# thunlp/OpenMatch

Hardware: NVIDIA H100
Metric: queries/sec top-1000 over 8.8M x 768 corpus (higher is better)
Workload: dtype f16

## Files before the change

openmatch_b200/csrc/encoder.cu:

```cuda
#include <math.h>
#include <stdlib.h>
#include <string.h>

#include <algorithm>
#include <new>
#include <set>
#include <string>
#include <vector>

#include "common.h"
#include "gemm.cuh"

namespace om {

constexpr int kAttnCols = 64;
constexpr int kMaxL = 128;
constexpr int kMaxLongL = 512;
constexpr float kLog2e = 1.4426950408889634f;

__device__ __forceinline__ float rcp_approx(float x) {
  float y;
  asm("rcp.approx.ftz.f32 %0, %1;" : "=f"(y) : "f"(x));
  return y;
}
// ... 94 lines not shown
      store_direct(held, out, ldo, row, held_col, M);
      have = 0;
    }
  }
  __device__ __forceinline__ void finish() {
    if (in_flight && (threadIdx.x & 31) == 0) bulk_wait_group0();
  }
};

template <int ACT>
struct EpiBiasActBf16 {
  CUtensorMap tm_out;
  __nv_bfloat16* out;
  int64_t ldo;
  const float* bias;
  int M, N;
  RowNorm norm;
  static constexpr int kPasses = 1;
  static constexpr bool kPrefetch = false;
  __host__ __device__ static constexpr int smem_bytes(int epi_warps) { return epi_warps * StagedBf16::kBytesPerWarp; }
  struct State {
    StagedBf16 stage;
    float rstd, rm;
  };
  __device__ __forceinline__ void bind(State& s, uint8_t* smem, int epi_tid) const { s.stage.bind(smem, epi_tid); }
  __device__ __forceinline__ void finish(State& s) const { s.stage.finish(); }
  __device__ __forceinline__ void begin(State& s, int row, int, int) const {
    s.stage.have = 0;
    norm.get(row, M, s.rstd, s.rm);
  }
  __device__ __forceinline__ void end(State& s, int row) const { s.stage.flush_tail(out, ldo, row, M); }
  __device__ __forceinline__ void chunk(State& s, int row, int col0, const float (&v)[32]) const {
    if (col0 >= N) return;
    uint32_t packed[16];
    float bv[32];
#pragma unroll
    for (int j = 0; j < 8; ++j) {
      const float4 t = bias ? __ldg(reinterpret_cast<const float4*>(bias + col0) + j) : make_float4(0.f, 0.f, 0.f, 0.f);
      bv[4 * j] = t.x, bv[4 * j + 1] = t.y, bv[4 * j + 2] = t.z, bv[4 * j + 3] = t.w;
    }
    const float2 rs = splat2(s.rstd);
#pragma unroll
    for (int i = 0; i < 32; i += 2) {
      float2 ab = fma2(rs, make_float2(v[i], v[i + 1]), make_float2(bv[i], bv[i + 1]));
      if (ACT == ACT_GELU) {
        ab = gelu_erf2(ab);
      } else if (ACT == ACT_RELU) {
        ab.x = fmaxf(ab.x, 0.f);
        ab.y = fmaxf(ab.y, 0.f);
      }
      packed[i >> 1] = pack_bf16x2(ab.x, ab.y);
    }
    s.stage.push(packed, &tm_out, row, col0);
  }
};

struct EpiQKV {
  CUtensorMap tm_qk;
  __nv_bfloat16* qk;
  __nv_bfloat16* vt;
  int64_t ldv;
  const float* bias;
  int M, I2;
  int valid_rows;
  RowNorm norm;
  static constexpr int kPasses = 1;
  static constexpr bool kPrefetch = false;
  __host__ __device__ static constexpr int smem_bytes(int epi_warps) { return epi_warps * StagedBf16::kBytesPerWarp; }
  struct State {
    int vcol;
    StagedBf16 stage;
    float rstd, rm;
  };
  __device__ __forceinline__ void bind(State& s, uint8_t* smem, int epi_tid) const { s.stage.bind(smem, epi_tid); }
  __device__ __forceinline__ void finish(State& s) const { s.stage.finish(); }
  __device__ __forceinline__ void begin(State& s, int row, int, int) const {
    s.vcol = (row / valid_rows) * 128 + row % valid_rows;
    s.stage.have = 0;
    norm.get(row, M, s.rstd, s.rm);
  }
  __device__ __forceinline__ void end(State& s, int row) const { s.stage.flush_tail(qk, I2, row, M); }
  __device__ __forceinline__ void chunk(State& s, int row, int col0, const float (&v)[32]) const {
    if (col0 >= I2 + (I2 >> 1)) return;
    float bv[32];
#pragma unroll
    for (int j = 0; j < 8; ++j) {
      const float4 t = bias ? __ldg(reinterpret_cast<const float4*>(bias + col0) + j) : make_float4(0.f, 0.f, 0.f, 0.f);
      bv[4 * j] = t.x, bv[4 * j + 1] = t.y, bv[4 * j + 2] = t.z, bv[4 * j + 3] = t.w;
    }
    const float rstd = s.rstd;
    if (col0 < I2) {
      uint32_t packed[16];
#pragma unroll
      for (int i = 0; i < 32; i += 2)
        packed[i >> 1] = pack_bf16x2(fmaf(rstd, v[i], bv[i]), fmaf(rstd, v[i + 1], bv[i + 1]));
      s.stage.push(packed, &tm_qk, row, col0);
    } else if (row < M) {
      __nv_bfloat16* dst = vt + static_cast<int64_t>(col0 - I2) * ldv + s.vcol;
#pragma unroll
      for (int i = 0; i < 32; ++i)
        dst[static_cast<int64_t>(i) * ldv] = __float2bfloat16(fmaf(rstd, v[i], bv[i]));
    }
  }
};

struct EpiResidNorm {
  CUtensorMap tm_s;
  CUtensorMap tm_xb;
  const float* bias;
  RowNorm norm;
  const float* gamma;
  const float* beta;
  float* stats_out;
  int parts;
  int M, N;
  int bn;
  static constexpr int kPasses = 1;
  static constexpr bool kPrefetch = true;
  static constexpr int kF32Tile = 4096, kBf16Tile = 2048, kPerWarp = kF32Tile + kBf16Tile;
  static constexpr int kMaxN = 1024;
  __host__ __device__ static constexpr int smem_bytes(int epi_warps) { return epi_warps * kPerWarp + 1024 + 2 * kMaxN * 4; }
  struct State {
    uint8_t* f32tile;
    uint8_t* bf16tile;
    uint64_t* bars;
    const float* gsm;
    const float* bsm;
    uint32_t parity;
    int slot;
    int group;
    float rstd, rm, rsum, rsq;
  };
  __device__ __forceinline__ void bind(State& s, uint8_t* smem, int epi_tid) const {
    const int w = epi_tid >> 5, nw = blockDim.x / 32 - kGemmProducerThreads / 32;
    s.f32tile = smem + w * kF32Tile;
    s.bf16tile = smem + nw * kF32Tile + w * kBf16Tile;
    s.bars = reinterpret_cast<uint64_t*>(smem + nw * kPerWarp) + w;
    s.parity = 0;
    s.group = w >> 2;
    if ((epi_tid & 31) == 0) {
      mbar_init(&s.bars[0], 1);
      fence_barrier_init();
    }
    float* gs = reinterpret_cast<float*>(smem + nw * kPerWarp + 1024);
    float* bs = gs + kMaxN;
    const bool ln = norm.stats != nullptr;
    for (int c = epi_tid; c < N; c += nw * 32) {
      gs[c] = ln ? gamma[c] : 1.f;
      bs[c] = (bias ? bias[c] : 0.f) + (ln ? beta[c] : 0.f);
    }
    s.gsm = gs;
    s.bsm = bs;
    named_bar_sync(1, nw * 32);
  }
  __device__ __forceinline__ void finish(State&) const {
    if ((threadIdx.x & 31) == 0) bulk_wait_group0();
  }
  __device__ __forceinline__ void begin(State& s, int row, int m_blk, int n_blk) const {
    norm.get(row, M, s.rstd, s.rm);
    s.rsum = 0.f;
    s.rsq = 0.f;
    s.slot = n_blk * parts + s.group;
    if (bn > 0 && (threadIdx.x & 31) == 0) {
      const int num_n = (N + bn - 1) / bn, num_m = (M + kBlockM - 1) / kBlockM;
      const int next = m_blk * num_n + n_blk + static_cast<int>(gridDim.x);
      if (next < num_m * num_n) {
        const int nm = next / num_n, nn = next - nm * num_n;
        const int row0 = row + (nm - m_blk) * kBlockM;
        const int cols = bn / parts;
#pragma unroll 1
        for (int c = 0; c < cols; c += 32) tma_prefetch_l2_2d(&tm_s, nn * bn + s.group * cols + c, row0);
      }
    }
  }
  __device__ __forceinline__ void request(State& s, int row0, int col0) const {
    bulk_wait_group_read0();
    mbar_arrive_expect_tx(&s.bars[0], kF32Tile);
    tma_load_2d(s.f32tile, &tm_s, &s.bars[0], col0, row0);
  }
  __device__ __forceinline__ void prefetch(State& s, int row, int col0) const {
    if (col0 >= N) return;
    if ((threadIdx.x & 31) == 0) request(s, row, col0);
  }
  __device__ __forceinline__ void end(State& s, int row) const {
    if (row < M)
      *reinterpret_cast<float2*>(stats_out + (static_cast<int64_t>(row) * kStatParts + s.slot) * 2) = make_float2(s.rsum, s.rsq);
  }
  __device__ __forceinline__ void chunk(State& s, int row, int col0, const float (&v)[32], int next_col0) const {
    if (col0 >= N) return;
    const int lane = threadIdx.x & 31;
    mbar_wait_warp(&s.bars[0], s.parity, 20);
    s.parity ^= 1u;
    uint8_t* mine = s.f32tile + lane * 128;
    uint8_t* mineb = s.bf16tile + lane * 64;
    const float rstd = s.rstd, nrm = -s.rm;
    const float4* gp = reinterpret_cast<const float4*>(s.gsm + col0);
    const float4* bp = reinterpret_cast<const float4*>(s.bsm + col0);
    float rsum = 0.f, rsq = 0.f;
#pragma unroll
    for (int p = 0; p < 8; ++p) {
      float4* slot = reinterpret_cast<float4*>(mine + ((p ^ (lane & 7)) << 4));
      const float4 r = *slot;
      const float4 g = gp[p], bb = bp[p];
      float4 o;
      o.x = fmaf(r.x, rstd * g.x, fmaf(nrm, g.x, bb.x)) + v[4 * p];
      o.y = fmaf(r.y, rstd * g.y, fmaf(nrm, g.y, bb.y)) + v[4 * p + 1];
      o.z = fmaf(r.z, rstd * g.z, fmaf(nrm, g.z, bb.z)) + v[4 * p + 2];
      o.w = fmaf(r.w, rstd * g.w, fmaf(nrm, g.w, bb.w)) + v[4 * p + 3];
      *slot = o;
      rsum += (o.x + o.y) + (o.z + o.w);
      rsq = fmaf(o.x, o.x, fmaf(o.y, o.y, fmaf(o.z, o.z, fmaf(o.w, o.w, rsq))));
      uint2* hb = reinterpret_cast<uint2*>(mineb + ((((p >> 1) ^ ((lane >> 1) & 3)) << 4) | ((p & 1) << 3)));
      *hb = make_uint2(pack_bf16x2(o.x, o.y), pack_bf16x2(o.z, o.w));
    }
    if (row < M) {
      s.rsum += rsum;
      s.rsq += rsq;
    }
    fence_proxy_async_smem();
    __syncwarp();
    if (lane == 0) {
      tma_store_2d(&tm_s, s.f32tile, col0, row);
      tma_store_2d(&tm_xb, s.bf16tile, col0, row);
      bulk_commit_group();
      if (next_col0 >= 0 && next_col0 < N) request(s, row, next_col0);
    }
  }
};

constexpr int kMaxVec = 8;

template <bool RMS>
__device__ __forceinline__ void norm_row(float4 (&v)[kMaxVec], int nvec, int H, float eps) {
  float s = 0.f;
  if (!RMS) {
#pragma unroll
    for (int j = 0; j < kMaxVec; ++j)
      if (j < nvec) s += (v[j].x + v[j].y) + (v[j].z + v[j].w);
#pragma unroll
    for (int o = 16; o > 0; o >>= 1) s += __shfl_xor_sync(0xffffffffu, s, o);
  }
  const float mean = RMS ? 0.f : s / H;
  float q = 0.f;
#pragma unroll
  for (int j = 0; j < kMaxVec; ++j)
    if (j < nvec) {
      const float a = v[j].x - mean, b = v[j].y - mean, c = v[j].z - mean, d = v[j].w - mean;
      q += (a * a + b * b) + (c * c + d * d);
    }
#pragma unroll
  for (int o = 16; o > 0; o >>= 1) q += __shfl_xor_sync(0xffffffffu, q, o);
  const float rstd = rsqrtf(q / H + eps);
#pragma unroll
  for (int j = 0; j < kMaxVec; ++j)
// ... 917 lines not shown
  if (kind == OM_DEVICE) OM_CUDA(cudaDeviceSynchronize());
  float* staged = dst_f32;
  float* tmp = nullptr;
  if (!staged) {
    OM_CUDA(cudaMalloc(&tmp, count * sizeof(float)));
    staged = tmp;
  }
  cudaError_t err =
      cudaMemcpy(staged, data, count * sizeof(float), kind == OM_HOST ? cudaMemcpyHostToDevice : cudaMemcpyDeviceToDevice);
  if (err == cudaSuccess && dst_bf16) {
    f32_to_bf16_kernel<<<static_cast<int>(std::min<size_t>((count + 255) / 256, 4096)), 256>>>(staged, dst_bf16,
                                                                                              (int64_t)count);
    err = cudaGetLastError();
  }
  if (err == cudaSuccess) err = cudaDeviceSynchronize();
  if (tmp) cudaFree(tmp);
  if (err != cudaSuccess) return fail(OM_ECUDA, "weight upload failed: %s", cudaGetErrorString(err));
  return 0;
}

template <int DH>
cudaError_t attn_opt_in() {
  const auto smem = cudaFuncAttributeMaxDynamicSharedMemorySize;
  cudaError_t err = cudaFuncSetAttribute(attn_stream_kernel<DH>, smem, kAttnStreamSmemBytes);
  if (err == cudaSuccess) err = cudaFuncSetAttribute(attn_long_kernel<DH>, smem, kAttnLongSmemBytes);
  if (err == cudaSuccess) err = cudaFuncSetAttribute(attn_kernel<DH>, smem, kAttnSmemBytes);
  return err;
}

template <int DH>
void attn_launch(const CUtensorMap& tmQK, const CUtensorMap& tmVt, const AttnParams& ap_long, int n_stream,
                 const CUtensorMap& tmQKl, const CUtensorMap& tmVtl, const AttnParams& apl, int n_long,
                 const AttnParams& ap_short, int n_short, int units, int sms, cudaStream_t st) {
  if (n_stream > 0)
    attn_stream_kernel<DH><<<dim3(n_stream, units), kAttnStreamThreads, kAttnStreamSmemBytes, st>>>(tmQK, tmVt, ap_long);
  if (n_long > 0) attn_long_kernel<DH><<<dim3(n_long, units), 128, kAttnLongSmemBytes, st>>>(tmQKl, tmVtl, apl);
  if (n_short > 0)
    attn_kernel<DH><<<std::min(n_short * units, sms * kAttnCtasPerSm), 128, kAttnSmemBytes, st>>>(tmQK, tmVt, ap_short,
                                                                                                 n_short, units);
}

int encode_layers(om_encoder* e, int T, const AttnParams& ap_long, int n_stream, int n_long, const AttnParams& ap_short,
                  int n_short, int sms, cudaStream_t st) {
  const om_encoder_desc& d = e->d;
  const int H = d.hidden, I = e->I, F = d.ffn;
  const bool bert = bert_like(d.arch);
  const int rows4 = (T + 3) / 4;
  const int n_tiles = n_stream + n_long + n_short;
  CUtensorMap tmQK, tmVt;
  if (make_tmap_bf16_2d(&tmQK, e->qk, (uint64_t)2 * I, (uint64_t)T, (uint64_t)2 * I * 2, 64, 128) != 0 ||
      make_tmap_bf16_2d(&tmVt, e->vt, (uint64_t)n_tiles * 128, (uint64_t)I, (uint64_t)e->Tld * 2, 64, 64) != 0)
    return fail(OM_ECUDA, "om_encode: tensor map creation failed");
  CUtensorMap tmQKl = tmQK, tmVtl = tmVt;
  AttnParams apl = ap_long;
  if (n_stream > 0 && n_long > 0) {
    const int off = n_stream * 128;
    if (make_tmap_bf16_2d(&tmQKl, e->qk + (size_t)off * 2 * I, (uint64_t)2 * I, (uint64_t)(T - off), (uint64_t)2 * I * 2,
                          64, 128) != 0 ||
        make_tmap_bf16_2d(&tmVtl, e->vt + off, (uint64_t)(n_tiles - n_stream) * 128, (uint64_t)I, (uint64_t)e->Tld * 2,
                          64, 64) != 0)
      return fail(OM_ECUDA, "om_encode: tensor map creation failed");
    apl.T = T - off;
    apl.kmask += off;
    apl.ctx += (size_t)off * I;
    apl.rowmap += off;
  }

  CUtensorMap tmQKout, tmInter, tmS, tmXb;
  if (make_tmap_bf16_2d(&tmQKout, e->qk, (uint64_t)2 * I, (uint64_t)T, (uint64_t)2 * I * 2, 64, 32) != 0 ||
      make_tmap_bf16_2d(&tmInter, e->inter, (uint64_t)F, (uint64_t)T, (uint64_t)F * 2, 64, 32) != 0 ||
      make_tmap_2d(&tmS, e->h, 4, (uint64_t)H, (uint64_t)T, (uint64_t)H * 4, 32, 32, 128) != 0 ||
      make_tmap_2d(&tmXb, e->xb, 2, (uint64_t)H, (uint64_t)T, (uint64_t)H * 2, 32, 32, 64) != 0)
    return fail(OM_ECUDA, "om_encode: output tensor map creation failed");
  const float inv_h = 1.0f / static_cast<float>(H);
  const int rms = bert ? 0 : 1;
  const RowNorm normA{e->stats[0], inv_h, d.ln_eps, rms}, normB{e->stats[1], inv_h, d.ln_eps, rms};
  const RowNorm ident{nullptr, inv_h, d.ln_eps, rms};
  auto wide_gemm = [&](const __nv_bfloat16* A, int K, const __nv_bfloat16* W, int M, int N, const auto& epi) -> cudaError_t {
    return launch_gemm<128, 3, false>(A, K, W, K, M, N, K, epi, sms, st);
  };
  auto resid_gemm = [&](const __nv_bfloat16* A, int K, const __nv_bfloat16* W, const EpiResidNorm& epi) -> cudaError_t {
    return launch_gemm<128, 3, false>(A, K, W, K, T, H, K, epi, sms, st);
  };
  if (((H + 127) / 128) * 2 > kStatParts)
    return fail(OM_EINVAL, "om_encode: hidden=%d needs more statistics slots than kStatParts", H);
  for (int li = 0; li < d.layers; ++li) {
    const LayerW& w = e->layers[li];
    NvtxRange nvtx_layer("om.encode.layer");
    const float* g_in = bert ? (li == 0 ? e->emb_g : e->layers[li - 1].ln2_g) : nullptr;
    const float* b_in = bert ? (li == 0 ? e->emb_b : e->layers[li - 1].ln2_b) : nullptr;
    {
      EpiQKV epi{tmQKout, e->qk, e->vt, e->Tld, bert ? w.bqkv_fold : nullptr, T, 2 * I, ap_short.Tvalid_rows, normA};
      cudaError_t err = wide_gemm(e->xb, H, w.wqkv, T, 3 * I, epi);
      if (err != cudaSuccess) return fail(OM_ECUDA, "QKV GEMM launch failed: %s", cudaGetErrorString(err));
    }
    const int units = I / kAttnCols;
    (e->dh == 64 ? attn_launch<64> : attn_launch<32>)(tmQK, tmVt, ap_long, n_stream, tmQKl, tmVtl, apl, n_long, ap_short,
                                                      n_short, units, sms, st);
    OM_CUDA(cudaGetLastError());
    {
      EpiResidNorm epi{tmS, tmXb, bert ? w.bo : nullptr, bert ? normA : ident, g_in, b_in, e->stats[1], 2, T, H, 128};
      cudaError_t err = resid_gemm(e->ctx, I, w.wo, epi);
      if (err != cudaSuccess) return fail(OM_ECUDA, "O-proj GEMM launch failed: %s", cudaGetErrorString(err));
    }
    {
      cudaError_t err;
      if (bert) {
        EpiBiasActBf16<ACT_GELU> epi{tmInter, e->inter, F, w.b1_fold, T, F, normB};
        err = wide_gemm(e->xb, H, w.w1, T, F, epi);
      } else {
        EpiBiasActBf16<ACT_RELU> epi{tmInter, e->inter, F, nullptr, T, F, normB};
        err = wide_gemm(e->xb, H, w.w1, T, F, epi);
      }
      if (err != cudaSuccess) return fail(OM_ECUDA, "FFN1 GEMM launch failed: %s", cudaGetErrorString(err));
    }
    {
      EpiResidNorm epi{tmS, tmXb, bert ? w.b2 : nullptr, bert ? normB : ident, w.ln1_g, w.ln1_b, e->stats[0], 2, T, H, 128};
      cudaError_t err = resid_gemm(e->inter, F, w.w2, epi);
      if (err != cudaSuccess) return fail(OM_ECUDA, "FFN2 GEMM launch failed: %s", cudaGetErrorString(err));
    }
  }
  if (bert)
    norm_kernel<false><<<rows4, 128, 0, st>>>(e->h, e->layers[d.layers - 1].ln2_g, e->layers[d.layers - 1].ln2_b,
                                              d.ln_eps, T, H, e->h);
  else
    norm_kernel<true><<<rows4, 128, 0, st>>>(e->h, e->final_g, nullptr, d.ln_eps, T, H, e->h);
  OM_CUDA(cudaGetLastError());
  return 0;
}

int embed_rows(om_encoder* e, const int64_t* ids, const int64_t* tts, int T, int L, const PackedSeq* seqs, int nseq,
               cudaStream_t st) {
  const om_encoder_desc& d = e->d;
  const int H = d.hidden, rows4 = (T + 3) / 4, type_vocab = std::max(d.type_vocab, 1);
  const int2* rowmap = seqs ? e->rowmap : nullptr;
  const int Lrow = seqs ? kMaxL : L;
  if (d.arch == OM_ARCH_ROBERTA) {
    roberta_pos_kernel<<<(nseq + 3) / 4, 128, 0, st>>>(ids, nseq, L, seqs, e->pos_ids);
    bert_embed_kernel<true><<<rows4, 128, 0, st>>>(ids, tts, e->word, e->type, e->pos, T, Lrow, H, d.vocab, type_vocab,
                                                   e->h, e->xb, e->stats[0], rowmap, seqs, e->pos_ids);
  } else if (d.arch == OM_ARCH_BERT) {
    bert_embed_kernel<false><<<rows4, 128, 0, st>>>(ids, tts, e->word, e->type, e->pos, T, Lrow, H, d.vocab, type_vocab,
                                                    e->h, e->xb, e->stats[0], rowmap, seqs, nullptr);
  } else {
    t5_embed_kernel<<<rows4, 128, 0, st>>>(ids, e->word, T, H, d.vocab, e->h, e->xb, e->stats[0], rowmap, seqs);
  }
  OM_CUDA(cudaGetLastError());
  return 0;
}

int check_out(const om_encoder* e, const char* who, const void* out_reps, om_dtype out_dtype, int64_t out_row_stride) {
  if (!out_reps) return fail(OM_EINVAL, "%s: null argument", who);
  if (!e->finalized) return fail(OM_ESTATE, "%s: call om_encoder_finalize first", who);
  if (out_dtype != OM_F32 && out_dtype != OM_BF16 && out_dtype != OM_F16)
    return fail(OM_EINVAL, "%s: out dtype must be f32, bf16 or f16", who);
  if (out_row_stride < om_encoder_rep_dim(e)) return fail(OM_EINVAL, "%s: out_row_stride < rep_dim", who);
  return 0;
}

float attn_scale_log2(const om_encoder* e) {
  const float scale = bert_like(e->d.arch) ? static_cast<float>(1.0 / sqrt(static_cast<double>(e->dh))) : 1.0f;
  return scale * kLog2e;
}

int finish_reps(om_encoder* e, int B, void* out_reps, om_dtype out_dtype, int64_t out_row_stride, cudaStream_t st) {
  const om_encoder_desc& d = e->d;
  const int H = d.hidden, rep_dim = om_encoder_rep_dim(e);
  const float* reps = e->pooled;
  if (d.has_head) {
    const int warps = d.head_out * ((B + 7) / 8);
    head_kernel<<<(warps * 32 + 255) / 256, 256, 0, st>>>(e->pooled, e->head_w, B, H, d.head_out, e->headed);
    reps = e->headed;
  }
  if (out_dtype == OM_F32)
    finish_reps_kernel<float><<<(B + 3) / 4, 128, 0, st>>>(reps, B, rep_dim, d.normalize, static_cast<float*>(out_reps),
                                                          out_row_stride);
  else if (out_dtype == OM_BF16)
    finish_reps_kernel<__nv_bfloat16><<<(B + 3) / 4, 128, 0, st>>>(reps, B, rep_dim, d.normalize,
                                                                  static_cast<__nv_bfloat16*>(out_reps), out_row_stride);
  else
    finish_reps_kernel<__half><<<(B + 3) / 4, 128, 0, st>>>(reps, B, rep_dim, d.normalize, static_cast<__half*>(out_reps),
                                                           out_row_stride);
  OM_CUDA(cudaGetLastError());
  return 0;
}

struct PackedGroup {
  int k0, k1;
  int T;
  int n_stream;
  int n_long;
  int n_tiles;
};

void place_packed(const int32_t* len, const int64_t* tok0, int n, int Tmax, std::vector<PackedSeq>& seqs,
                  std::vector<PackedGroup>& groups) {
  seqs.clear();
  groups.clear();
  const int cap = std::min(kMaxL, Tmax);
  std::vector<int> streams, longs, shorts;
// ... 500 lines not shown
```

openmatch_b200/csrc/gemm.cuh:

```cuda
#pragma once
#include <type_traits>

#include "ring.cuh"
#include "tmap.cuh"

namespace om {

constexpr int kBlockM = 128;
constexpr int kBlockK = 64;
constexpr int kWgmmaK = 16;
constexpr int kGemmProducerThreads = 128;
constexpr int kGemmEpiWarps = 8;

template <int BN, int STAGES>
struct GemmCfg {
  static_assert(BN == 128, "BN must be 128 (one wgmma m64n128 per consumer warpgroup)");
  static constexpr int kABytes = kBlockM * kBlockK * 2;
  static constexpr int kBBytes = BN * kBlockK * 2;
  static constexpr int kStageBytes = kABytes + kBBytes;
  static constexpr int kAccPitch = BN + 4;
  static constexpr int kAccOffset = STAGES * kStageBytes;
  static constexpr int kBarOffset = kAccOffset + kBlockM * kAccPitch * 4;
  static constexpr int kEpiOffset = kBarOffset + 1024;
  static constexpr int kSmemBytes = kEpiOffset + 1024;
  static_assert(kBarOffset % 1024 == 0, "barrier block must stay 1024-B aligned");
};


template <int BN, bool F16>
__device__ __forceinline__ void wgmma_tile_k16(float (&acc)[BN / 2], uint64_t da, uint64_t db, uint32_t accumulate) {
  if constexpr (F16) wgmma_m64n128k16_f16<0, 0>(acc, da, db, accumulate);
  else wgmma_m64n128k16_bf16<0, 0>(acc, da, db, accumulate);
}

template <int BN, int STAGES, bool M_FASTEST, class Epi, bool F16>
__global__ void __launch_bounds__(kGemmProducerThreads + 32 * kGemmEpiWarps, 1)
gemm_bf16_tn_kernel(const __grid_constant__ CUtensorMap tmA, const __grid_constant__ CUtensorMap tmB, int M, int N,
                    int K, const __grid_constant__ Epi epi, int* tile_counter) {
  using Cfg = GemmCfg<BN, STAGES>;
  extern __shared__ uint8_t smem_raw[];
  uint8_t* smem = reinterpret_cast<uint8_t*>((reinterpret_cast<uintptr_t>(smem_raw) + 1023) & ~uintptr_t(1023));
  float* acc_tile = reinterpret_cast<float*>(smem + Cfg::kAccOffset);
  uint64_t* full_bar = reinterpret_cast<uint64_t*>(smem + Cfg::kBarOffset);
  uint64_t* empty_bar = full_bar + STAGES;
  constexpr int kSched = 4;
  uint64_t* sfull_bar = empty_bar + STAGES;
  uint64_t* sempty_bar = sfull_bar + kSched;
  volatile int* tile_ring = reinterpret_cast<volatile int*>(sempty_bar + kSched);
  uint8_t* epi_smem = smem + Cfg::kEpiOffset;
  const bool dyn = tile_counter != nullptr;

  const int warp = __shfl_sync(0xffffffffu, static_cast<int>(threadIdx.x >> 5), 0);
  const int lane = static_cast<int>(threadIdx.x & 31);

  if (warp == 0 && lane == 0) {
    tma_prefetch_desc(&tmA);
    tma_prefetch_desc(&tmB);
  }
  if (warp == 1 && lane == 0) {
    ring_init(full_bar, empty_bar, STAGES, kGemmEpiWarps);
    ring_init(sfull_bar, sempty_bar, kSched, kGemmEpiWarps);
    fence_barrier_init();
  }
  __syncthreads();

  const int num_m = (M + kBlockM - 1) / kBlockM;
  const int num_n = (N + BN - 1) / BN;
  const int num_tiles = num_m * num_n;
  const int num_k = (K + kBlockK - 1) / kBlockK;
  const int first_tile = static_cast<int>(blockIdx.x);
  const int tile_step = static_cast<int>(gridDim.x);

  if (warp == 0) {
    if (lane == 0) {
      Ring<STAGES> ring;
      Ring<kSched> sched;
      int tile = first_tile;
      if (dyn) {
        tile = atomicAdd(tile_counter, 1);
        if (tile >= num_tiles) tile = -1;
      }
      while (true) {
        if (dyn) {
          ring_wait_free(sempty_bar, sched, 5);
          tile_ring[sched.stage] = tile;
          mbar_arrive(&sfull_bar[sched.stage]);
          sched.advance();
          if (tile < 0) break;
        } else if (tile >= num_tiles) {
          break;
        }
        int next = dyn ? atomicAdd(tile_counter, 1) : tile + tile_step;
        const int m_blk = M_FASTEST ? tile % num_m : tile / num_n;
        const int n_blk = M_FASTEST ? tile / num_m : tile % num_n;
        for (int kb = 0; kb < num_k; ++kb) {
          uint64_t* bar = ring_acquire_tx(full_bar, empty_bar, ring, Cfg::kStageBytes, 1);
          uint8_t* sa = smem + ring.stage * Cfg::kStageBytes;
          tma_load_2d(sa, &tmA, bar, kb * kBlockK, m_blk * kBlockM);
          tma_load_2d(sa + Cfg::kABytes, &tmB, bar, kb * kBlockK, n_blk * BN);
          ring.advance();
        }
        tile = (dyn && next >= num_tiles) ? -1 : next;
      }
    }
  } else if (warp >= 4) {
    const int et = static_cast<int>(threadIdx.x) - kGemmProducerThreads;
    const int wg = et >> 7;
    const int ew = (warp - 4) & 3;
    const int half = (warp - 4) >> 2;
    constexpr int kChunks = BN / 32 / 2;
    typename Epi::State st;
    if constexpr (Epi::smem_bytes(kGemmEpiWarps) > 0) epi.bind(st, epi_smem, et);
    Ring<kSched> sched;
    Ring<STAGES> ring;
    const int frow = 64 * wg + 16 * (warp & 3) + (lane >> 2), fcol = 2 * (lane & 3);
    for (int tile = first_tile;; tile += tile_step) {
      if (dyn) {
        mbar_wait_warp(&sfull_bar[sched.stage], sched.phase, 7);
        tile = tile_ring[sched.stage];
        __syncwarp();
        if (lane == 0) mbar_arrive(&sempty_bar[sched.stage]);
        sched.advance();
        if (tile < 0) break;
      } else if (tile >= num_tiles) {
        break;
      }
      const int m_blk = M_FASTEST ? tile % num_m : tile / num_n;
      const int n_blk = M_FASTEST ? tile / num_m : tile % num_n;
      const int row = m_blk * kBlockM + ew * 32 + lane;
      epi.begin(st, row, m_blk, n_blk);
      if constexpr (Epi::kPrefetch) epi.prefetch(st, row, n_blk * BN + half * kChunks * 32);

      float acc[BN / 2];
#pragma unroll
      for (int i = 0; i < BN / 2; ++i) acc[i] = 0.f;
      ring_consume(
          full_bar, ring, 0, num_k, 3,
          [&](uint32_t stage, uint32_t accumulate) {
            const uint32_t a_addr = smem_u32(smem + stage * Cfg::kStageBytes) + wg * (64 * 128);
            const uint32_t b_addr = smem_u32(smem + stage * Cfg::kStageBytes + Cfg::kABytes);
#pragma unroll
            for (int k = 0; k < kBlockK / kWgmmaK; ++k)
              wgmma_tile_k16<BN, F16>(acc, wgmma_desc(a_addr + k * 32, kDescKMajorSW128),
                                      wgmma_desc(b_addr + k * 32, kDescKMajorSW128), (accumulate | k) != 0 ? 1u : 0u);
          },
          [&](uint32_t stage) {
            if (lane == 0) mbar_arrive(&empty_bar[stage]);
          });
      wgmma_fence_regs(acc);

      named_bar_sync(2, 32 * kGemmEpiWarps);
#pragma unroll
      for (int j = 0; j < BN / 8; ++j) {
        *reinterpret_cast<float2*>(acc_tile + frow * Cfg::kAccPitch + 8 * j + fcol) = make_float2(acc[4 * j], acc[4 * j + 1]);
        *reinterpret_cast<float2*>(acc_tile + (frow + 8) * Cfg::kAccPitch + 8 * j + fcol) =
            make_float2(acc[4 * j + 2], acc[4 * j + 3]);
      }
      named_bar_sync(2, 32 * kGemmEpiWarps);

      const float* my_row = acc_tile + (ew * 32 + lane) * Cfg::kAccPitch;
#pragma unroll 1
      for (int pass = 0; pass < Epi::kPasses; ++pass) {
        if constexpr (Epi::kPasses > 1) {
          if (pass > 0) {
            if (!epi.need_pass(st, pass)) break;
            epi.between(st, row);
          }
        }
        const int c0 = half * kChunks;
#pragma unroll 1
        for (int c = c0; c < c0 + kChunks; ++c) {
          float v[32];
#pragma unroll
          for (int i = 0; i < 8; ++i) {
            const float4 t = *reinterpret_cast<const float4*>(my_row + c * 32 + 4 * i);
            v[4 * i] = t.x, v[4 * i + 1] = t.y, v[4 * i + 2] = t.z, v[4 * i + 3] = t.w;
          }
          const bool has_next = c + 1 < c0 + kChunks;
          if constexpr (Epi::kPasses > 1)
            epi.chunk(st, row, n_blk * BN + c * 32, v, pass);
          else if constexpr (Epi::kPrefetch)
            epi.chunk(st, row, n_blk * BN + c * 32, v, has_next ? n_blk * BN + (c + 1) * 32 : -1);
          else
            epi.chunk(st, row, n_blk * BN + c * 32, v);
        }
      }
      epi.end(st, row);
    }
    if constexpr (Epi::smem_bytes(kGemmEpiWarps) > 0) epi.finish(st);
  }

  __syncthreads();
}

static inline int* next_tile_counter(cudaStream_t stream) {
  static int* pool = nullptr;
  static unsigned next = 0;
  if (!pool && cudaMalloc(&pool, 64 * sizeof(int)) != cudaSuccess) return nullptr;
  int* c = pool + (next++ & 63u);
  if (cudaMemsetAsync(c, 0, sizeof(int), stream) != cudaSuccess) return nullptr;
  return c;
}

template <int BN, int STAGES, bool M_FASTEST, class Epi, bool F16 = false>
static inline cudaError_t launch_gemm(const void* A, int64_t lda, const void* B, int64_t ldb, int M, int N, int K,
                                      const Epi& epi, int num_sms, cudaStream_t stream, bool dynamic_sched = false) {
  using Cfg = GemmCfg<BN, STAGES>;
  if (M <= 0 || N <= 0 || K <= 0) return cudaSuccess;
  CUtensorMap tmA, tmB;
  if (make_tmap_bf16_2d(&tmA, A, (uint64_t)K, (uint64_t)M, (uint64_t)lda * 2, kBlockK, kBlockM) != 0)
    return cudaErrorInvalidValue;
  if (make_tmap_bf16_2d(&tmB, B, (uint64_t)K, (uint64_t)N, (uint64_t)ldb * 2, kBlockK, BN) != 0)
    return cudaErrorInvalidValue;
  auto kern = gemm_bf16_tn_kernel<BN, STAGES, M_FASTEST, Epi, F16>;
  const int smem_bytes = Cfg::kSmemBytes + Epi::smem_bytes(kGemmEpiWarps);
  static bool attr_set = false;
  if (!attr_set) {
    cudaError_t e = cudaFuncSetAttribute(kern, cudaFuncAttributeMaxDynamicSharedMemorySize, smem_bytes);
    if (e != cudaSuccess) return e;
    attr_set = true;
  }
  const int num_tiles = ((M + kBlockM - 1) / kBlockM) * ((N + BN - 1) / BN);
  const int threads = kGemmProducerThreads + 32 * kGemmEpiWarps;
  const int grid = num_tiles < num_sms ? num_tiles : num_sms;
  int* counter = nullptr;
  if (dynamic_sched) {
    counter = next_tile_counter(stream);
    if (!counter) return cudaErrorMemoryAllocation;
  }
  kern<<<grid, threads, smem_bytes, stream>>>(tmA, tmB, M, N, K, epi, counter);
  return cudaGetLastError();
}

}
```

Measured before the change: 39110.

## Ping-pong consumer warpgroups so one tile's epilogue overlaps the other's MMA

Each consumer warpgroup now owns a whole 128x128 tile, issuing two m64n128 wgmmas per k-step, and the two warpgroups alternate tiles. Order and staging mbarriers serialize their MMA issue and shared accumulator-tile use. The goal is to hide epilogue time behind the peer warpgroup's tensor-core work. Register reallocation (setmaxnreg) gives consumers more registers for the doubled accumulators, and the residual-norm epilogue drops its two-part statistics split. The cost is extra barrier complexity, and one warpgroup must skip ring stages to stay in sync.

```diff
diff --git a/openmatch_b200/csrc/encoder.cu b/openmatch_b200/csrc/encoder.cu
--- a/openmatch_b200/csrc/encoder.cu
+++ b/openmatch_b200/csrc/encoder.cu
@@ -230,7 +230,6 @@
   const float* gamma;
   const float* beta;
   float* stats_out;
-  int parts;
   int M, N;
   int bn;
   static constexpr int kPasses = 1;
@@ -246,7 +245,6 @@
     const float* bsm;
     uint32_t parity;
     int slot;
-    int group;
     float rstd, rm, rsum, rsq;
   };
   __device__ __forceinline__ void bind(State& s, uint8_t* smem, int epi_tid) const {
@@ -255,7 +253,6 @@
     s.bf16tile = smem + nw * kF32Tile + w * kBf16Tile;
     s.bars = reinterpret_cast<uint64_t*>(smem + nw * kPerWarp) + w;
     s.parity = 0;
-    s.group = w >> 2;
     if ((epi_tid & 31) == 0) {
       mbar_init(&s.bars[0], 1);
       fence_barrier_init();
@@ -278,16 +275,15 @@
     norm.get(row, M, s.rstd, s.rm);
     s.rsum = 0.f;
     s.rsq = 0.f;
-    s.slot = n_blk * parts + s.group;
+    s.slot = n_blk;
     if (bn > 0 && (threadIdx.x & 31) == 0) {
       const int num_n = (N + bn - 1) / bn, num_m = (M + kBlockM - 1) / kBlockM;
       const int next = m_blk * num_n + n_blk + static_cast<int>(gridDim.x);
       if (next < num_m * num_n) {
         const int nm = next / num_n, nn = next - nm * num_n;
         const int row0 = row + (nm - m_blk) * kBlockM;
-        const int cols = bn / parts;
 #pragma unroll 1
-        for (int c = 0; c < cols; c += 32) tma_prefetch_l2_2d(&tm_s, nn * bn + s.group * cols + c, row0);
+        for (int c = 0; c < bn; c += 32) tma_prefetch_l2_2d(&tm_s, nn * bn + c, row0);
       }
     }
   }
@@ -1371,7 +1367,7 @@
   auto resid_gemm = [&](const __nv_bfloat16* A, int K, const __nv_bfloat16* W, const EpiResidNorm& epi) -> cudaError_t {
     return launch_gemm<128, 3, false>(A, K, W, K, T, H, K, epi, sms, st);
   };
-  if (((H + 127) / 128) * 2 > kStatParts)
+  if ((H + 127) / 128 > kStatParts)
     return fail(OM_EINVAL, "om_encode: hidden=%d needs more statistics slots than kStatParts", H);
   for (int li = 0; li < d.layers; ++li) {
     const LayerW& w = e->layers[li];
@@ -1388,7 +1384,7 @@
                                                       n_short, units, sms, st);
     OM_CUDA(cudaGetLastError());
     {
-      EpiResidNorm epi{tmS, tmXb, bert ? w.bo : nullptr, bert ? normA : ident, g_in, b_in, e->stats[1], 2, T, H, 128};
+      EpiResidNorm epi{tmS, tmXb, bert ? w.bo : nullptr, bert ? normA : ident, g_in, b_in, e->stats[1], T, H, 128};
       cudaError_t err = resid_gemm(e->ctx, I, w.wo, epi);
       if (err != cudaSuccess) return fail(OM_ECUDA, "O-proj GEMM launch failed: %s", cudaGetErrorString(err));
     }
@@ -1404,7 +1400,7 @@
       if (err != cudaSuccess) return fail(OM_ECUDA, "FFN1 GEMM launch failed: %s", cudaGetErrorString(err));
     }
     {
-      EpiResidNorm epi{tmS, tmXb, bert ? w.b2 : nullptr, bert ? normB : ident, w.ln1_g, w.ln1_b, e->stats[0], 2, T, H, 128};
+      EpiResidNorm epi{tmS, tmXb, bert ? w.b2 : nullptr, bert ? normB : ident, w.ln1_g, w.ln1_b, e->stats[0], T, H, 128};
       cudaError_t err = resid_gemm(e->inter, F, w.w2, epi);
       if (err != cudaSuccess) return fail(OM_ECUDA, "FFN2 GEMM launch failed: %s", cudaGetErrorString(err));
     }
diff --git a/openmatch_b200/csrc/gemm.cuh b/openmatch_b200/csrc/gemm.cuh
--- a/openmatch_b200/csrc/gemm.cuh
+++ b/openmatch_b200/csrc/gemm.cuh
@@ -14,7 +14,7 @@
 
 template <int BN, int STAGES>
 struct GemmCfg {
-  static_assert(BN == 128, "BN must be 128 (one wgmma m64n128 per consumer warpgroup)");
+  static_assert(BN == 128, "BN must be 128 (two wgmma m64n128 per consumer warpgroup)");
   static constexpr int kABytes = kBlockM * kBlockK * 2;
   static constexpr int kBBytes = BN * kBlockK * 2;
   static constexpr int kStageBytes = kABytes + kBBytes;
@@ -46,7 +46,9 @@
   constexpr int kSched = 4;
   uint64_t* sfull_bar = empty_bar + STAGES;
   uint64_t* sempty_bar = sfull_bar + kSched;
-  volatile int* tile_ring = reinterpret_cast<volatile int*>(sempty_bar + kSched);
+  uint64_t* order_bar = sempty_bar + kSched;
+  uint64_t* staged_bar = order_bar + 2;
+  volatile int* tile_ring = reinterpret_cast<volatile int*>(staged_bar + 2);
   uint8_t* epi_smem = smem + Cfg::kEpiOffset;
   const bool dyn = tile_counter != nullptr;
 
@@ -58,8 +60,12 @@
     tma_prefetch_desc(&tmB);
   }
   if (warp == 1 && lane == 0) {
-    ring_init(full_bar, empty_bar, STAGES, kGemmEpiWarps);
+    ring_init(full_bar, empty_bar, STAGES, kGemmEpiWarps / 2);
     ring_init(sfull_bar, sempty_bar, kSched, kGemmEpiWarps);
+    for (int g = 0; g < 2; ++g) {
+      mbar_init(&order_bar[g], kGemmEpiWarps / 2);
+      mbar_init(&staged_bar[g], kGemmEpiWarps / 2);
+    }
     fence_barrier_init();
   }
   __syncthreads();
@@ -71,8 +77,9 @@
   const int first_tile = static_cast<int>(blockIdx.x);
   const int tile_step = static_cast<int>(gridDim.x);
 
-  if (warp == 0) {
-    if (lane == 0) {
+  if (warp < 4) {
+    setmaxnreg_dec<40>();
+    if (warp == 0 && lane == 0) {
       Ring<STAGES> ring;
       Ring<kSched> sched;
       int tile = first_tile;
@@ -103,60 +110,86 @@
         tile = (dyn && next >= num_tiles) ? -1 : next;
       }
     }
-  } else if (warp >= 4) {
+  } else {
+    setmaxnreg_inc<232>();
     const int et = static_cast<int>(threadIdx.x) - kGemmProducerThreads;
     const int wg = et >> 7;
     const int ew = (warp - 4) & 3;
-    const int half = (warp - 4) >> 2;
-    constexpr int kChunks = BN / 32 / 2;
+    constexpr int kChunks = BN / 32;
     typename Epi::State st;
     if constexpr (Epi::smem_bytes(kGemmEpiWarps) > 0) epi.bind(st, epi_smem, et);
     Ring<kSched> sched;
     Ring<STAGES> ring;
-    const int frow = 64 * wg + 16 * (warp & 3) + (lane >> 2), fcol = 2 * (lane & 3);
-    for (int tile = first_tile;; tile += tile_step) {
+    uint32_t order_phase = 0, staged_phase = 0;
+    auto read_sched = [&]() -> int {
+      mbar_wait_warp(&sfull_bar[sched.stage], sched.phase, 7);
+      const int t = tile_ring[sched.stage];
+      __syncwarp();
+      if (lane == 0) mbar_arrive(&sempty_bar[sched.stage]);
+      sched.advance();
+      return t;
+    };
+    const int frow = 16 * ew + (lane >> 2), fcol = 2 * (lane & 3);
+    int tile = first_tile + (wg - 2) * tile_step;
+    for (bool first = true;; first = false) {
+      const bool after_peer = !first || wg == 1;
       if (dyn) {
-        mbar_wait_warp(&sfull_bar[sched.stage], sched.phase, 7);
-        tile = tile_ring[sched.stage];
-        __syncwarp();
-        if (lane == 0) mbar_arrive(&sempty_bar[sched.stage]);
-        sched.advance();
+        if (after_peer && read_sched() < 0) break;
+        tile = read_sched();
         if (tile < 0) break;
-      } else if (tile >= num_tiles) {
-        break;
+      } else {
+        tile += 2 * tile_step;
+        if (tile >= num_tiles) break;
       }
       const int m_blk = M_FASTEST ? tile % num_m : tile / num_n;
       const int n_blk = M_FASTEST ? tile / num_m : tile % num_n;
       const int row = m_blk * kBlockM + ew * 32 + lane;
       epi.begin(st, row, m_blk, n_blk);
-      if constexpr (Epi::kPrefetch) epi.prefetch(st, row, n_blk * BN + half * kChunks * 32);
-
-      float acc[BN / 2];
-#pragma unroll
-      for (int i = 0; i < BN / 2; ++i) acc[i] = 0.f;
+      if constexpr (Epi::kPrefetch) epi.prefetch(st, row, n_blk * BN);
+
+      if (after_peer) {
+        for (int kb = 0; kb < num_k; ++kb) ring.advance();
+        mbar_wait_warp(&order_bar[wg], order_phase, 8);
+        order_phase ^= 1u;
+      }
+      float acc[2][BN / 2];
+#pragma unroll
+      for (int i = 0; i < BN / 2; ++i) acc[0][i] = acc[1][i] = 0.f;
+      int issued = 0;
       ring_consume(
           full_bar, ring, 0, num_k, 3,
           [&](uint32_t stage, uint32_t accumulate) {
-            const uint32_t a_addr = smem_u32(smem + stage * Cfg::kStageBytes) + wg * (64 * 128);
+            const uint32_t a_addr = smem_u32(smem + stage * Cfg::kStageBytes);
             const uint32_t b_addr = smem_u32(smem + stage * Cfg::kStageBytes + Cfg::kABytes);
 #pragma unroll
-            for (int k = 0; k < kBlockK / kWgmmaK; ++k)
-              wgmma_tile_k16<BN, F16>(acc, wgmma_desc(a_addr + k * 32, kDescKMajorSW128),
-                                      wgmma_desc(b_addr + k * 32, kDescKMajorSW128), (accumulate | k) != 0 ? 1u : 0u);
+            for (int k = 0; k < kBlockK / kWgmmaK; ++k) {
+              const uint64_t db = wgmma_desc(b_addr + k * 32, kDescKMajorSW128);
+              const uint32_t acc_on = (accumulate | k) != 0 ? 1u : 0u;
+              wgmma_tile_k16<BN, F16>(acc[0], wgmma_desc(a_addr + k * 32, kDescKMajorSW128), db, acc_on);
+              wgmma_tile_k16<BN, F16>(acc[1], wgmma_desc(a_addr + 64 * 128 + k * 32, kDescKMajorSW128), db, acc_on);
+            }
+            if (++issued == num_k && lane == 0) mbar_arrive(&order_bar[wg ^ 1]);
           },
           [&](uint32_t stage) {
             if (lane == 0) mbar_arrive(&empty_bar[stage]);
           });
-      wgmma_fence_regs(acc);
-
-      named_bar_sync(2, 32 * kGemmEpiWarps);
-#pragma unroll
-      for (int j = 0; j < BN / 8; ++j) {
-        *reinterpret_cast<float2*>(acc_tile + frow * Cfg::kAccPitch + 8 * j + fcol) = make_float2(acc[4 * j], acc[4 * j + 1]);
-        *reinterpret_cast<float2*>(acc_tile + (frow + 8) * Cfg::kAccPitch + 8 * j + fcol) =
-            make_float2(acc[4 * j + 2], acc[4 * j + 3]);
-      }
-      named_bar_sync(2, 32 * kGemmEpiWarps);
+      wgmma_fence_regs(acc[0]);
+      wgmma_fence_regs(acc[1]);
+
+      if (after_peer) {
+        mbar_wait_warp(&staged_bar[wg], staged_phase, 9);
+        staged_phase ^= 1u;
+      }
+#pragma unroll
+      for (int h = 0; h < 2; ++h) {
+#pragma unroll
+        for (int j = 0; j < BN / 8; ++j) {
+          float* r0 = acc_tile + (64 * h + frow) * Cfg::kAccPitch + 8 * j + fcol;
+          *reinterpret_cast<float2*>(r0) = make_float2(acc[h][4 * j], acc[h][4 * j + 1]);
+          *reinterpret_cast<float2*>(r0 + 8 * Cfg::kAccPitch) = make_float2(acc[h][4 * j + 2], acc[h][4 * j + 3]);
+        }
+      }
+      named_bar_sync(2 + wg, 128);
 
       const float* my_row = acc_tile + (ew * 32 + lane) * Cfg::kAccPitch;
 #pragma unroll 1
@@ -167,24 +200,24 @@
             epi.between(st, row);
           }
         }
-        const int c0 = half * kChunks;
 #pragma unroll 1
-        for (int c = c0; c < c0 + kChunks; ++c) {
+        for (int c = 0; c < kChunks; ++c) {
           float v[32];
 #pragma unroll
           for (int i = 0; i < 8; ++i) {
             const float4 t = *reinterpret_cast<const float4*>(my_row + c * 32 + 4 * i);
             v[4 * i] = t.x, v[4 * i + 1] = t.y, v[4 * i + 2] = t.z, v[4 * i + 3] = t.w;
           }
-          const bool has_next = c + 1 < c0 + kChunks;
           if constexpr (Epi::kPasses > 1)
             epi.chunk(st, row, n_blk * BN + c * 32, v, pass);
           else if constexpr (Epi::kPrefetch)
-            epi.chunk(st, row, n_blk * BN + c * 32, v, has_next ? n_blk * BN + (c + 1) * 32 : -1);
+            epi.chunk(st, row, n_blk * BN + c * 32, v, c + 1 < kChunks ? n_blk * BN + (c + 1) * 32 : -1);
           else
             epi.chunk(st, row, n_blk * BN + c * 32, v);
         }
       }
+      __syncwarp();
+      if (lane == 0) mbar_arrive(&staged_bar[wg ^ 1]);
       epi.end(st, row);
     }
     if constexpr (Epi::smem_bytes(kGemmEpiWarps) > 0) epi.finish(st);
```

Measured after the change: 39120, median of 6. Within noise of the previous version (+0.0%).

## Split GEMM consumers into separate MMA and epilogue warpgroups with mbarrier handoff

Applied to the files above, without the earlier changes.

The persistent GEMM kernel now has dedicated MMA warps and separate epilogue warps, with setmaxnreg used to rebalance registers between producer, MMA and epilogue roles. The two roles hand off the shared fp32 accumulator tile through acc_full/acc_empty mbarriers, so the next tile's wgmma can start while the epilogue drains the previous one. This replaces the named-barrier serialization. It also fuses the bias loads into the pack/store loops in the QKV epilogue to lower register pressure. It raises the thread count and uses a single acc tile buffer, so overlap is limited to the MMA main loop, and the encoder time may matter little for a retrieval query-rate metric.

```diff
diff --git a/openmatch_b200/csrc/encoder.cu b/openmatch_b200/csrc/encoder.cu
--- a/openmatch_b200/csrc/encoder.cu
+++ b/openmatch_b200/csrc/encoder.cu
@@ -200,24 +200,27 @@
   __device__ __forceinline__ void end(State& s, int row) const { s.stage.flush_tail(qk, I2, row, M); }
   __device__ __forceinline__ void chunk(State& s, int row, int col0, const float (&v)[32]) const {
     if (col0 >= I2 + (I2 >> 1)) return;
-    float bv[32];
-#pragma unroll
-    for (int j = 0; j < 8; ++j) {
-      const float4 t = bias ? __ldg(reinterpret_cast<const float4*>(bias + col0) + j) : make_float4(0.f, 0.f, 0.f, 0.f);
-      bv[4 * j] = t.x, bv[4 * j + 1] = t.y, bv[4 * j + 2] = t.z, bv[4 * j + 3] = t.w;
-    }
+    const float4* bias4 = reinterpret_cast<const float4*>(bias + col0);
     const float rstd = s.rstd;
     if (col0 < I2) {
       uint32_t packed[16];
 #pragma unroll
-      for (int i = 0; i < 32; i += 2)
-        packed[i >> 1] = pack_bf16x2(fmaf(rstd, v[i], bv[i]), fmaf(rstd, v[i + 1], bv[i + 1]));
+      for (int j = 0; j < 8; ++j) {
+        const float4 b = bias ? __ldg(bias4 + j) : make_float4(0.f, 0.f, 0.f, 0.f);
+        packed[2 * j] = pack_bf16x2(fmaf(rstd, v[4 * j], b.x), fmaf(rstd, v[4 * j + 1], b.y));
+        packed[2 * j + 1] = pack_bf16x2(fmaf(rstd, v[4 * j + 2], b.z), fmaf(rstd, v[4 * j + 3], b.w));
+      }
       s.stage.push(packed, &tm_qk, row, col0);
     } else if (row < M) {
       __nv_bfloat16* dst = vt + static_cast<int64_t>(col0 - I2) * ldv + s.vcol;
 #pragma unroll
-      for (int i = 0; i < 32; ++i)
-        dst[static_cast<int64_t>(i) * ldv] = __float2bfloat16(fmaf(rstd, v[i], bv[i]));
+      for (int j = 0; j < 8; ++j) {
+        const float4 b = bias ? __ldg(bias4 + j) : make_float4(0.f, 0.f, 0.f, 0.f);
+        dst[static_cast<int64_t>(4 * j) * ldv] = __float2bfloat16(fmaf(rstd, v[4 * j], b.x));
+        dst[static_cast<int64_t>(4 * j + 1) * ldv] = __float2bfloat16(fmaf(rstd, v[4 * j + 1], b.y));
+        dst[static_cast<int64_t>(4 * j + 2) * ldv] = __float2bfloat16(fmaf(rstd, v[4 * j + 2], b.z));
+        dst[static_cast<int64_t>(4 * j + 3) * ldv] = __float2bfloat16(fmaf(rstd, v[4 * j + 3], b.w));
+      }
     }
   }
 };
@@ -250,7 +253,7 @@
     float rstd, rm, rsum, rsq;
   };
   __device__ __forceinline__ void bind(State& s, uint8_t* smem, int epi_tid) const {
-    const int w = epi_tid >> 5, nw = blockDim.x / 32 - kGemmProducerThreads / 32;
+    const int w = epi_tid >> 5, nw = kGemmEpiWarps;
     s.f32tile = smem + w * kF32Tile;
     s.bf16tile = smem + nw * kF32Tile + w * kBf16Tile;
     s.bars = reinterpret_cast<uint64_t*>(smem + nw * kPerWarp) + w;
diff --git a/openmatch_b200/csrc/gemm.cuh b/openmatch_b200/csrc/gemm.cuh
--- a/openmatch_b200/csrc/gemm.cuh
+++ b/openmatch_b200/csrc/gemm.cuh
@@ -10,7 +10,15 @@
 constexpr int kBlockK = 64;
 constexpr int kWgmmaK = 16;
 constexpr int kGemmProducerThreads = 128;
+constexpr int kGemmMmaWarps = 8;
 constexpr int kGemmEpiWarps = 8;
+constexpr int kGemmThreads = kGemmProducerThreads + 32 * (kGemmMmaWarps + kGemmEpiWarps);
+constexpr int kGemmProducerRegs = 40;
+constexpr int kGemmMmaRegs = 96;
+constexpr int kGemmEpiRegs = 120;
+static_assert(kGemmProducerThreads * kGemmProducerRegs + 32 * (kGemmMmaWarps * kGemmMmaRegs + kGemmEpiWarps * kGemmEpiRegs) <=
+                  kGemmThreads * 96,
+              "register budgets exceed the launch allocation");
 
 template <int BN, int STAGES>
 struct GemmCfg {
@@ -34,7 +42,7 @@
 }
 
 template <int BN, int STAGES, bool M_FASTEST, class Epi, bool F16>
-__global__ void __launch_bounds__(kGemmProducerThreads + 32 * kGemmEpiWarps, 1)
+__global__ void __launch_bounds__(kGemmThreads, 1)
 gemm_bf16_tn_kernel(const __grid_constant__ CUtensorMap tmA, const __grid_constant__ CUtensorMap tmB, int M, int N,
                     int K, const __grid_constant__ Epi epi, int* tile_counter) {
   using Cfg = GemmCfg<BN, STAGES>;
@@ -46,7 +54,9 @@
   constexpr int kSched = 4;
   uint64_t* sfull_bar = empty_bar + STAGES;
   uint64_t* sempty_bar = sfull_bar + kSched;
-  volatile int* tile_ring = reinterpret_cast<volatile int*>(sempty_bar + kSched);
+  uint64_t* acc_full = sempty_bar + kSched;
+  uint64_t* acc_empty = acc_full + 1;
+  volatile int* tile_ring = reinterpret_cast<volatile int*>(acc_empty + 1);
   uint8_t* epi_smem = smem + Cfg::kEpiOffset;
   const bool dyn = tile_counter != nullptr;
 
@@ -58,8 +68,10 @@
     tma_prefetch_desc(&tmB);
   }
   if (warp == 1 && lane == 0) {
-    ring_init(full_bar, empty_bar, STAGES, kGemmEpiWarps);
-    ring_init(sfull_bar, sempty_bar, kSched, kGemmEpiWarps);
+    ring_init(full_bar, empty_bar, STAGES, kGemmMmaWarps);
+    ring_init(sfull_bar, sempty_bar, kSched, kGemmMmaWarps + kGemmEpiWarps);
+    mbar_init(acc_full, kGemmMmaWarps);
+    mbar_init(acc_empty, kGemmEpiWarps);
     fence_barrier_init();
   }
   __syncthreads();
@@ -70,9 +82,19 @@
   const int num_k = (K + kBlockK - 1) / kBlockK;
   const int first_tile = static_cast<int>(blockIdx.x);
   const int tile_step = static_cast<int>(gridDim.x);
-
-  if (warp == 0) {
-    if (lane == 0) {
+  auto next_tile = [&](Ring<kSched>& sched, int tile, uint32_t site) -> int {
+    if (!dyn) return tile < num_tiles ? tile : -1;
+    mbar_wait_warp(&sfull_bar[sched.stage], sched.phase, site);
+    tile = tile_ring[sched.stage];
+    __syncwarp();
+    if (lane == 0) mbar_arrive(&sempty_bar[sched.stage]);
+    sched.advance();
+    return tile;
+  };
+
+  if (warp < 4) {
+    setmaxnreg_dec<kGemmProducerRegs>();
+    if (warp == 0 && lane == 0) {
       Ring<STAGES> ring;
       Ring<kSched> sched;
       int tile = first_tile;
@@ -103,37 +125,20 @@
         tile = (dyn && next >= num_tiles) ? -1 : next;
       }
     }
-  } else if (warp >= 4) {
-    const int et = static_cast<int>(threadIdx.x) - kGemmProducerThreads;
-    const int wg = et >> 7;
-    const int ew = (warp - 4) & 3;
-    const int half = (warp - 4) >> 2;
-    constexpr int kChunks = BN / 32 / 2;
-    typename Epi::State st;
-    if constexpr (Epi::smem_bytes(kGemmEpiWarps) > 0) epi.bind(st, epi_smem, et);
+  } else if (warp < 4 + kGemmMmaWarps) {
+    setmaxnreg_inc<kGemmMmaRegs>();
+    const int wg = (warp - 4) >> 2;
     Ring<kSched> sched;
     Ring<STAGES> ring;
+    uint32_t acc_phase = 0;
     const int frow = 64 * wg + 16 * (warp & 3) + (lane >> 2), fcol = 2 * (lane & 3);
-    for (int tile = first_tile;; tile += tile_step) {
-      if (dyn) {
-        mbar_wait_warp(&sfull_bar[sched.stage], sched.phase, 7);
-        tile = tile_ring[sched.stage];
-        __syncwarp();
-        if (lane == 0) mbar_arrive(&sempty_bar[sched.stage]);
-        sched.advance();
-        if (tile < 0) break;
-      } else if (tile >= num_tiles) {
-        break;
-      }
-      const int m_blk = M_FASTEST ? tile % num_m : tile / num_n;
-      const int n_blk = M_FASTEST ? tile / num_m : tile % num_n;
-      const int row = m_blk * kBlockM + ew * 32 + lane;
-      epi.begin(st, row, m_blk, n_blk);
-      if constexpr (Epi::kPrefetch) epi.prefetch(st, row, n_blk * BN + half * kChunks * 32);
+    for (int i = first_tile;; i += tile_step) {
+      const int tile = next_tile(sched, i, 7);
+      if (tile < 0) break;
 
       float acc[BN / 2];
 #pragma unroll
-      for (int i = 0; i < BN / 2; ++i) acc[i] = 0.f;
+      for (int j = 0; j < BN / 2; ++j) acc[j] = 0.f;
       ring_consume(
           full_bar, ring, 0, num_k, 3,
           [&](uint32_t stage, uint32_t accumulate) {
@@ -149,16 +154,38 @@
           });
       wgmma_fence_regs(acc);
 
-      named_bar_sync(2, 32 * kGemmEpiWarps);
+      mbar_wait_warp(acc_empty, acc_phase ^ 1u, 8);
 #pragma unroll
       for (int j = 0; j < BN / 8; ++j) {
         *reinterpret_cast<float2*>(acc_tile + frow * Cfg::kAccPitch + 8 * j + fcol) = make_float2(acc[4 * j], acc[4 * j + 1]);
         *reinterpret_cast<float2*>(acc_tile + (frow + 8) * Cfg::kAccPitch + 8 * j + fcol) =
             make_float2(acc[4 * j + 2], acc[4 * j + 3]);
       }
-      named_bar_sync(2, 32 * kGemmEpiWarps);
-
-      const float* my_row = acc_tile + (ew * 32 + lane) * Cfg::kAccPitch;
+      __syncwarp();
+      if (lane == 0) mbar_arrive(acc_full);
+      acc_phase ^= 1u;
+    }
+  } else {
+    setmaxnreg_inc<kGemmEpiRegs>();
+    const int et = static_cast<int>(threadIdx.x) - (kGemmProducerThreads + 32 * kGemmMmaWarps);
+    const int ew = (et >> 5) & 3;
+    const int half = et >> 7;
+    constexpr int kChunks = BN / 32 / 2;
+    typename Epi::State st;
+    if constexpr (Epi::smem_bytes(kGemmEpiWarps) > 0) epi.bind(st, epi_smem, et);
+    Ring<kSched> sched;
+    uint32_t acc_phase = 0;
+    const float* my_row = acc_tile + (ew * 32 + lane) * Cfg::kAccPitch;
+    for (int i = first_tile;; i += tile_step) {
+      const int tile = next_tile(sched, i, 11);
+      if (tile < 0) break;
+      const int m_blk = M_FASTEST ? tile % num_m : tile / num_n;
+      const int n_blk = M_FASTEST ? tile / num_m : tile % num_n;
+      const int row = m_blk * kBlockM + ew * 32 + lane;
+      epi.begin(st, row, m_blk, n_blk);
+      if constexpr (Epi::kPrefetch) epi.prefetch(st, row, n_blk * BN + half * kChunks * 32);
+
+      mbar_wait_warp(acc_full, acc_phase, 9);
 #pragma unroll 1
       for (int pass = 0; pass < Epi::kPasses; ++pass) {
         if constexpr (Epi::kPasses > 1) {
@@ -172,9 +199,9 @@
         for (int c = c0; c < c0 + kChunks; ++c) {
           float v[32];
 #pragma unroll
-          for (int i = 0; i < 8; ++i) {
-            const float4 t = *reinterpret_cast<const float4*>(my_row + c * 32 + 4 * i);
-            v[4 * i] = t.x, v[4 * i + 1] = t.y, v[4 * i + 2] = t.z, v[4 * i + 3] = t.w;
+          for (int j = 0; j < 8; ++j) {
+            const float4 t = *reinterpret_cast<const float4*>(my_row + c * 32 + 4 * j);
+            v[4 * j] = t.x, v[4 * j + 1] = t.y, v[4 * j + 2] = t.z, v[4 * j + 3] = t.w;
           }
           const bool has_next = c + 1 < c0 + kChunks;
           if constexpr (Epi::kPasses > 1)
@@ -185,6 +212,9 @@
             epi.chunk(st, row, n_blk * BN + c * 32, v);
         }
       }
+      __syncwarp();
+      if (lane == 0) mbar_arrive(acc_empty);
+      acc_phase ^= 1u;
       epi.end(st, row);
     }
     if constexpr (Epi::smem_bytes(kGemmEpiWarps) > 0) epi.finish(st);
@@ -221,14 +251,13 @@
     attr_set = true;
   }
   const int num_tiles = ((M + kBlockM - 1) / kBlockM) * ((N + BN - 1) / BN);
-  const int threads = kGemmProducerThreads + 32 * kGemmEpiWarps;
-  const int grid = num_tiles < num_sms ? num_tiles : num_sms;
+    const int grid = num_tiles < num_sms ? num_tiles : num_sms;
   int* counter = nullptr;
   if (dynamic_sched) {
     counter = next_tile_counter(stream);
     if (!counter) return cudaErrorMemoryAllocation;
   }
-  kern<<<grid, threads, smem_bytes, stream>>>(tmA, tmB, M, N, K, epi, counter);
+  kern<<<grid, kGemmThreads, smem_bytes, stream>>>(tmA, tmB, M, N, K, epi, counter);
   return cudaGetLastError();
 }
 
```

Result: no change. 38650 before, 38750 after (median of 6 runs) (+0.3%).
